# LockedFlysher/optimal_control_problem

Measured on AMD Instinct MI355X. Metric: QP solves/sec (batched OSQP-ADMM, N=20), higher is better.
Workload: dtype f64

## Files before the change

### __graft_entry__.py

```python
import os
import subprocess
import sys

ROOT = os.path.dirname(os.path.abspath(__file__))
if ROOT not in sys.path:
    sys.path.insert(0, ROOT)


def _run(cmd):
    subprocess.check_call(cmd, cwd=ROOT, stdout=subprocess.DEVNULL)


def _stale(target, deps):
    return (not os.path.exists(target)) or any(os.path.getmtime(d) > os.path.getmtime(target) for d in deps)


def build():
    pk = os.path.join(ROOT, "optimal_control_problem_amd")
    so = os.path.join(pk, "libmpcqp.so")
    cdir = os.path.join(pk, "csrc")
    csrc = [os.path.join(cdir, f) for f in sorted(os.listdir(cdir)) if f.endswith((".hip", ".hpp")) or f == "Makefile"]
    if _stale(so, csrc + [os.path.join(ROOT, "include", "mpcqp.h")]):
        _run(["make", "-C", cdir, "-j", str(min(8, os.cpu_count() or 1)), "../libmpcqp.so"])
    orc = os.path.join(ROOT, "oracle", "liborc.so")
    if _stale(orc, [os.path.join(ROOT, "oracle", "osqp_oracle.c"), os.path.join(ROOT, "oracle", "osqp_oracle.h")]):
        _run(["make", "-C", os.path.join(ROOT, "oracle"), "-B", "liborc.so"])
    pi = os.path.join(ROOT, "tests", "support", "libplan_interp.so")
    if _stale(pi, [os.path.join(ROOT, "tests", "support", "plan_interp.cpp"), os.path.join(pk, "csrc", "plan.hpp"), os.path.join(pk, "csrc", "select.hpp")]):
        _run(["g++", "-O2", "-std=c++17", "-fPIC", "-shared", "-o", pi, os.path.join(ROOT, "tests", "support", "plan_interp.cpp")])
    sm = os.path.join(ROOT, "tests", "support", "libstage_models_host.so")
    if _stale(sm, [os.path.join(ROOT, "tests", "support", "stage_models_host.cpp"), os.path.join(pk, "csrc", "stage_models.hpp")]):
        _run(["g++", "-O2", "-std=c++17", "-ffp-contract=off", "-fPIC", "-shared", "-o", sm, os.path.join(ROOT, "tests", "support", "stage_models_host.cpp")])
    st = os.path.join(ROOT, "tests", "support", "libstage_tracking_host.so")
    if _stale(st, [os.path.join(ROOT, "tests", "support", "stage_tracking_host.cpp"), os.path.join(pk, "csrc", "stage_models.hpp")]):
        _run(["g++", "-O2", "-std=c++17", "-ffp-contract=off", "-fPIC", "-shared", "-o", st, os.path.join(ROOT, "tests", "support", "stage_tracking_host.cpp")])
    sl_ = os.path.join(ROOT, "tests", "support", "libstage_link_cost_host.so")
    if _stale(sl_, [os.path.join(ROOT, "tests", "support", "stage_link_cost_host.cpp"), os.path.join(pk, "csrc", "stage_models.hpp")]):
        _run(["g++", "-O2", "-std=c++17", "-ffp-contract=off", "-fPIC", "-shared", "-o", sl_, os.path.join(ROOT, "tests", "support", "stage_link_cost_host.cpp")])
    cv = os.path.join(ROOT, "tests", "support", "libconvexify_host.so")
    if _stale(cv, [os.path.join(ROOT, "tests", "support", "convexify_host.cpp"), os.path.join(pk, "csrc", "stage_convexify.hpp"),
                   os.path.join(pk, "csrc", "stage_models.hpp"), os.path.join(ROOT, "include", "mpcqp.h")]):
        _run(["g++", "-O2", "-std=c++17", "-ffp-contract=off", "-fPIC", "-shared", "-o", cv, os.path.join(ROOT, "tests", "support", "convexify_host.cpp")])
    cpp = os.path.join(ROOT, "tests", "support", "cucaqp_cpp_test")
    src = os.path.join(ROOT, "tests", "support", "cucaqp_cpp_test.cpp")
# ... 84 lines not shown
```

### optimal_control_problem_amd/csrc/kernel_oc_rescale.hpp

```cpp
#pragma once

template <int NW, bool HUB>
__global__ void __launch_bounds__(NW * WAVE, 2) mpcqp_oc_rescale_kernel(const DevPlan pl, const DevRes rs, const mpcqp_settings st, const DevIO io, const DevOc oc) {
  extern __shared__ __attribute__((aligned(16))) double lds[];
  constexpr int NT = NW * WAVE;
  const int lane = threadIdx.x & 63;
  const int b = __builtin_amdgcn_readfirstlane(io.order ? io.order[blockIdx.x] : (int)blockIdx.x);
  int wid = __builtin_amdgcn_readfirstlane(threadIdx.x >> 6);
  if constexpr (NW == 4) wid = oc_wave_role4(lds, wid, lane, io.no_remap);
  const int tid = wid * WAVE + lane;
  const OcLds<NW> L = oc_lds<NW, true>(lds, pl, rs, oc);
  RCtx cx;
  cx.pl = &pl; cx.rs = &rs; cx.st = &st; cx.wid = wid; cx.lane = lane;
  cx.fts[0] = cx.fts[1] = cx.fts[2] = cx.fts[3] = 0;
  double *ws = io.ws + (long)b * pl.ws_stride; cx.ws = ws;
  cx.BL = ws + pl.o_Lf; cx.TMP = lds;
  cx.X = L.X; cx.Q = L.Q; cx.R = L.R; cx.Z = L.Z; cx.Y = L.Y; cx.W = L.W; cx.RB = L.RB; cx.RED = L.RED;
  double *valA = ws + pl.o_ellA, *valAt = ws + pl.o_ellAt, *valP = ws + pl.o_ellP;
  double *lb = ws + pl.o_l, *ub = ws + pl.o_u, *Qs = ws + pl.o_Lb;
  const double *Dg = ws + pl.o_D, *Eg = ws + pl.o_E;
  const double *inP = io.P + (long)b * io.sP, *inA = io.A + (long)b * io.sA, *inq = io.q + (long)b * io.sq;
  const double *inl = io.l + (long)b * io.sl, *inu = io.u + (long)b * io.su;
  const int n = pl.n, m = pl.m, npad = pl.npad, mpad = pl.mpad;
  cx.unscale = st.scaling && !st.scaled_termination;
// ... 12 lines not shown
    const int i = ch * WAVE + lane; const double ei = i < mpad ? cx.W[i] : 0.0;
    ell_map_chunk<true>(valA, pl.A.src, inA, pl.A.idx, valA, cx.coA[ch], cx.coA[ch + 1], lane, [&](double v, int j) { return v * (ei * cx.R[j]); });
  }
  for (int ch = wid; ch < pl.At.nchunks; ch += NW) {
    const int t = ch * WAVE + lane; const double dj = t < npad ? cx.R[t] : 0.0;
    ell_map_chunk<true>(valAt, pl.At.src, inA, pl.At.idx, valAt, cx.coAt[ch], cx.coAt[ch + 1], lane, [&](double v, int i) { return v * (dj * cx.W[i]); });
  }
  for (int ch = wid; ch < pl.P.nchunks; ch += NW) {
    const int t = ch * WAVE + lane; const double dj = t < npad ? cx.R[t] : 0.0;
    ell_map_chunk<true>(valP, pl.P.src, inP, pl.P.idx, valP, cx.coP[ch], cx.coP[ch + 1], lane, [&](double v, int k) { return v * (c * dj * cx.R[k]); });
  }
  bsync<NW>();
  double rho = io.info[4L * b + 3];
  if (!(rho >= Q_RHO_MIN && rho <= Q_RHO_MAX)) rho = fmin(fmax(st.rho, Q_RHO_MIN), Q_RHO_MAX);
  cx.rho = uni(rho);
  const bool ok = factorize_res<NW, (HUB ? 2 : 1), false>(cx, &oc, L.octab, lds);
  if (tid == 0) {
    io.status[b] = ok ? MPCQP_UNSOLVED : MPCQP_NON_CVX; io.iters[b] = 0;
    io.info[4L * b + 3] = cx.rho;
  }
}
```

### optimal_control_problem_amd/csrc/kernel_oc_split.hpp

```cpp
#pragma once

constexpr int OC_PENDING = 100, OC_PENDING_NONCVX = 101;
template <int NW>
struct OcLds {
  double *X, *Q, *R, *Z, *Y, *W, *RB, *RED;
  int *octab, *co;
};
template <int NW, bool SETUP = false>
__device__ __forceinline__ OcLds<NW> oc_lds(double *lds, const DevPlan &pl, const DevRes &rs, const DevOc &oc) {
  OcLds<NW> L;
  L.X = lds + rs.stage; L.Q = L.X + pl.npad; L.R = SETUP ? L.Q : L.Q + pl.npad;
  double *rend = L.R + pl.npad + rs.rext;
  L.Z = rend; L.Y = L.Z + (SETUP ? oc.zpad : pl.mpad); L.W = L.Y + (SETUP ? pl.npad : pl.mpad);
  L.RB = L.W + pl.mpad; L.RED = L.RB + 16 * NW + 16;
  L.octab = reinterpret_cast<int *>(L.RED + 16 * NW) + 8;
  L.co = L.octab + ((oc.o_pos + 1) & ~1);
  return L;
}
__device__ __forceinline__ int oc_wave_role4(double *lds, int wid, const int lane, const int no_remap) {
  const unsigned hw = __builtin_amdgcn_s_getreg((31 << 11) | 4), la = __builtin_amdgcn_s_getreg((31 << 11) | 6);
  const int simd = (hw >> 4) & 3, slot = (la & 0xff) != 0;
  int *xs = reinterpret_cast<int *>(lds);
  if (lane == 0) xs[wid] = simd;
  bsync<4>();
// ... 52 lines not shown
  double *lb = ws + pl.o_l, *ub = ws + pl.o_u, *Dg = ws + pl.o_D, *Eg = ws + pl.o_E, *Qs = ws + pl.o_Lb;
  const double *inP = io.P + (long)b * io.sP, *inA = io.A + (long)b * io.sA, *inq = io.q + (long)b * io.sq;
  const double *inl = io.l + (long)b * io.sl, *inu = io.u + (long)b * io.su;
  const int n = pl.n, m = pl.m, npad = pl.npad, mpad = pl.mpad;
  cx.unscale = st.scaling && !st.scaled_termination;
  TS_DECL;
#ifdef MPCQP_TIMING_RUIZ
  unsigned long long rzacc[5] = {0, 0, 0, 0, 0};
#endif
  if (oc.resume && io.status[b] != OC_PENDING) return;
  oc_tables_to_lds<NW>(pl, oc, cx, L, tid);
  if (oc.resume) {
    bsync<NW>();
    cx.rho = uni(io.info[4L * b + 3]);
    cx.c = 1.0; cx.cinv = 1.0;
    const bool okr = factorize_res<NW, (HUB ? 2 : 1), false>(cx, &oc, L.octab, lds);
    if (tid == 0) io.status[b] = okr ? OC_PENDING : OC_PENDING_NONCVX;
    return;
  }
  double c = 1.0;
  int refactor = 1, prev_status = MPCQP_UNSOLVED;
  const bool reuse = REUSE && io.reuse;
  if (reuse) {
    prev_status = io.status[b];
    c = io.cscale[b];
    for (int t = tid; t < npad; t += NT) { if (pl.perm[t] < 0) Qs[t] = 0.0; cx.R[t] = Dg[t]; }
    bsync<NW>();
    for (int j = tid; j < n; j += NT) { const int t = pl.pos[j]; Qs[t] = inq[j] * (c * cx.R[t]); }
    double chg[1] = {0.0};
    for (int i = tid; i < mpad; i += NT) {
      const double ei = Eg[i];
// ... 163 lines not shown
    };
    unsigned short *iA16 = reinterpret_cast<unsigned short *>(lds) + oc.ixo_a, *iP16 = reinterpret_cast<unsigned short *>(lds) + oc.ixo_p;
    constexpr std::false_type plain{}; constexpr std::true_type regs{};
    if (a_lds && p_lds && oc.ix16 == 3) scale_phase(lds, lds + pl.A.entries, iA16, iP16, plain);
    else if (a_lds && p_lds && oc.ix16 == 1) scale_phase(lds, lds + pl.A.entries, iA16, pl.P.idx, plain);
    else if (a_lds && p_lds) scale_phase(lds, lds + pl.A.entries, pl.A.idx, pl.P.idx, plain);
    else if (a_lds) scale_phase(lds, valP, pl.A.idx, pl.P.idx, regs);
    else if (oc.ix16 == 3) scale_phase(valA, valP, iA16, iP16, regs);
    else if (oc.ix16 == 1) scale_phase(valA, valP, iA16, pl.P.idx, regs);
    else scale_phase(valA, valP, pl.A.idx, pl.P.idx, regs);
  }
  bsync<NW>();
  cx.rho = uni(reuse ? io.info[4L * b + 3] : fmin(fmax(io.rho0 && io.rho0[b] > 0.0 ? io.rho0[b] : st.rho, Q_RHO_MIN), Q_RHO_MAX));
  TS(2);
  bool ok = !(reuse && prev_status == MPCQP_NON_CVX);
  if (ok && refactor) ok = factorize_res<NW, (HUB ? 2 : 1), false>(cx, &oc, L.octab, lds);
  if (tid == 0) {
    io.status[b] = ok ? MPCQP_UNSOLVED : MPCQP_NON_CVX; io.iters[b] = 0;
    io.info[4L * b + 3] = cx.rho;
    io.cscale[b] = c;
  }
  TS(3);
#ifdef MPCQP_TIMING
  ts_acc[12] = cx.fts[0]; ts_acc[13] = cx.fts[1]; ts_acc[14] = cx.fts[2]; ts_acc[15] = cx.fts[3];
#ifdef MPCQP_TIMING_RUIZ
  ts_acc[9] = rzacc[0]; ts_acc[10] = rzacc[1]; ts_acc[11] = rzacc[2]; ts_acc[12] = rzacc[3]; ts_acc[13] = rzacc[4];
#endif
#endif
  TS_STORE(io.dbg);
}

// ... 329 lines not shown
```

### optimal_control_problem_amd/csrc/kernel_onchip.hpp

```cpp
#pragma once

struct DevTile {
  int on, ntile;
  int nAr, nAtr;
  const int *Ar_off, *Ar_idx, *Ar_src, *Atr_off, *Atr_idx, *Atr_src;
  long Ar_entries, Atr_entries;
  const int *tJ, *rowid, *tsrc;
  const int *ta_info, *ta_cnt;
  const unsigned long long *ta_mask;
  const int *tt_info;
  long o_tile, o_ellAr, o_ellAtr;
};
struct DevOc {
  int nbc, has_hub, junc, npw, nhr, nlds, ntab;
  int o_chainE, o_chainF, o_pos, o_fill, ghub_slot, ghub_src;
  const int *a_assign;
  int npair, o_pair;
  int nfill, o_s, o_dbl, ndbl, o_pp;
  int at_poll, at_free;
  int a_lds, p_lds;
  const int *tab;
  const int *asm_rec;
  DevTile tl;
  int resume;
  int ixo_a, ixo_p;
  int ix16, zpad;
  int no_ruiz_regs = 0;
};

__host__ __device__ __forceinline__ int oc_swz(int r, int c) {
  return ((r ^ ((r >> 2) & 1)) << 4) | (c ^ (((r >> 1) & 3) << 2) ^ (((r >> 3) & 1) << 1));
}

typedef double d2 __attribute__((ext_vector_type(2)));

struct OcLane {
  unsigned f4;
  unsigned t4;
  int k4;
  int o4;
};
__device__ __forceinline__ OcLane oc_lane(int lane) {
  OcLane ln;
// ... 811 lines not shown
```

### optimal_control_problem_amd/csrc/kernel_resident.hpp

```cpp
#pragma once

#ifdef MPCQP_TIMING
#define TS_DECL unsigned long long ts_last = __builtin_amdgcn_s_memtime(), ts_acc[16] = {0}; const unsigned long long ts_first = ts_last, ts_rt0 = __builtin_amdgcn_s_memrealtime()
#define TS(k) do { unsigned long long t_ = __builtin_amdgcn_s_memtime(); ts_acc[k] += t_ - ts_last; ts_last = t_; } while (0)
#define TS_STORE(ptr) do { if (tid == 0 && (ptr)) { for (int k_ = 0; k_ < 16; k_++) (ptr)[16L * b + k_] = (long long)ts_acc[k_]; \
    if (b == 0) { (ptr)[16L * gridDim.x + 126] = (long long)(__builtin_amdgcn_s_memtime() - ts_first); (ptr)[16L * gridDim.x + 127] = (long long)(__builtin_amdgcn_s_memrealtime() - ts_rt0); } } } while (0)
#else
#define TS_DECL
#ifdef MPCQP_ASM_MARKS
#define TS(k) do { __builtin_amdgcn_sched_barrier(0); asm volatile("; TS " #k ::: "memory"); } while (0)
#else
#define TS(k) __builtin_amdgcn_sched_barrier(0)
#endif
#define TS_STORE(ptr)
#endif
struct DevRes {
  int nphase, ntemp, nconst, rext;
  const int *lv_ptr, *lv_diag, *lw_ptr, *lw_slot, *lw_g, *lu_ptr, *lu_dst, *lu_tmp, *lu_b, *g_ptr, *g_seg;
  int n_seg, nlev; long stage;
  int tmp_alias;
};


struct RCtx {
// ... 347 lines not shown
  t.i[0] = __builtin_amdgcn_mov_dpp(a.i[0], 0xB1, 0xF, 0xF, true);
  t.i[1] = __builtin_amdgcn_mov_dpp(a.i[1], 0xB1, 0xF, 0xF, true);
  a.d += t.d;
  t.i[0] = __builtin_amdgcn_mov_dpp(a.i[0], 0x4E, 0xF, 0xF, true);
  t.i[1] = __builtin_amdgcn_mov_dpp(a.i[1], 0x4E, 0xF, 0xF, true);
  return a.d + t.d;
}

__device__ __forceinline__ d4 mfma_abt_l(const double *A, const double *B, d4 acc, int lane) {
  const int rr = lane & 15, kk = lane >> 4;
#pragma unroll
  for (int k0 = 0; k0 < BS; k0 += 4) {
    const double a = A[rr * BS + k0 + kk];
    const double b = B[rr * BS + k0 + kk];
    acc = __builtin_amdgcn_mfma_f64_16x16x4f64(a, b, acc, 0, 0, 0);
  }
  return acc;
}

template <bool T>
__device__ __forceinline__ d4 load_blk(const char *BLb, const int off, const int offN, const int offT) {
  if (T) {
    const char *B = BLb + off + offT;
    d4 r;
    r[0] = *reinterpret_cast<const double *>(B); r[1] = *reinterpret_cast<const double *>(B + BS * 8);
    r[2] = *reinterpret_cast<const double *>(B + 2 * BS * 8); r[3] = *reinterpret_cast<const double *>(B + 3 * BS * 8);
    return r;
  }
  return *reinterpret_cast<const d4 *>(BLb + off + offN);
}
// ... 130 lines not shown
#pragma unroll
  for (int u = 0; u < U; u++) { v[u] = vp[u * WAVE]; fl[u] = fp[u * WAVE]; ix[u] = ip[u * WAVE]; }
#pragma unroll
  for (int u = 0; u < U; u++) if (fl[u]) acc += w[ix[u]] * v[u] * v[u];
  vp += U * WAVE; fp += U * WAVE; ip += U * WAVE;
}
template <int U>
__device__ __forceinline__ void tscatter_batch(const double *&vp, const int *&tp, double *T, const double sr) {
  double v[U]; int t[U];
#pragma unroll
  for (int u = 0; u < U; u++) { v[u] = vp[u * WAVE]; t[u] = tp[u * WAVE]; }
#pragma unroll
  for (int u = 0; u < U; u++) if (t[u] >= 0) T[t[u]] = v[u] * sr;
  vp += U * WAVE; tp += U * WAVE;
}
template <int NW, int OCM = 0, bool TAIL = true>
__device__ __forceinline__ bool factorize_res(RCtx &cx, const DevOc *oc = nullptr, const int *octab = nullptr, double *scr = nullptr) {
  const DevPlan &pl = *cx.pl; const DevRes &rs = *cx.rs; double *ws = cx.ws;
  const int wid = cx.wid, lane = cx.lane, tid = wid * WAVE + lane; constexpr int NT = NW * WAVE;
  const double *lb = ws + pl.o_l, *ub = ws + pl.o_u;
  const double *valA = ws + pl.o_ellA, *valAt = ws + pl.o_ellAt, *valP = ws + pl.o_ellP;
  double *T = ws + pl.o_T;
#ifdef MPCQP_TIMING
  unsigned long long f0 = __builtin_amdgcn_s_memtime();
#endif
  for (int i = tid; i < pl.mpad; i += NT) cx.W[i] = i < pl.m ? rho_of(lb[i], ub[i], cx.rho) : 0.0;
  bsync<NW>();
  {
    const double sigma = cx.st->sigma;
    const DevEll &E = pl.At;
    for (int c = wid; c < E.nchunks; c += NW) {
      double acc = 0.0;
      const int s0 = cx.coAt[c], s1 = cx.coAt[c + 1];
      const long o = (long)s0 * WAVE + lane;
      const double *vp = valAt + o; const int *fp = E.flag + o, *ip = E.idx + o;
      int rem = s1 - s0;
      for (; rem >= 8; rem -= 8) dvec_batch<8>(vp, fp, ip, cx.W, acc);
      if (rem & 4) dvec_batch<4>(vp, fp, ip, cx.W, acc);
      if (rem & 2) dvec_batch<2>(vp, fp, ip, cx.W, acc);
      if (rem & 1) dvec_batch<1>(vp, fp, ip, cx.W, acc);
      const int t = c * WAVE + lane;
      if (t < pl.npad) cx.R[t] = pl.perm[t] >= 0 ? sigma + acc : 1.0;
    }
  }
  {
    const DevEll &E = pl.A;
    for (int c = wid; c < E.nchunks; c += NW) {
      const int i = c * WAVE + lane;
      const double sr = sqrt(cx.W[i]);
      const int s0 = cx.coA[c], s1 = cx.coA[c + 1];
      const long o = (long)s0 * WAVE + lane;
      const double *vp = valA + o; const int *tp = pl.tpos + o;
      int rem = s1 - s0;
      for (; rem >= 8; rem -= 8) tscatter_batch<8>(vp, tp, T, sr);
      if (rem & 4) tscatter_batch<4>(vp, tp, T, sr);
      if (rem & 2) tscatter_batch<2>(vp, tp, T, sr);
      if (rem & 1) tscatter_batch<1>(vp, tp, T, sr);
    }
  }
  int *rec = nullptr;
  if constexpr (OCM > 0) {
    rec = reinterpret_cast<int *>(scr + OC_LDL_SCR * BLK);
    for (int k = tid; k < 8 * pl.nblk; k += NT) rec[k] = oc->asm_rec[k];
  }
  bsync<NW>();
#ifdef MPCQP_TIMING
  unsigned long long f1 = __builtin_amdgcn_s_memtime(); cx.fts[0] += f1 - f0;
#endif
  const int row0 = lane >> 4, col = lane & 15;
  if constexpr (OCM > 0) {
    const int nblk = pl.nblk;
    auto rfl = [](int v) { return __builtin_amdgcn_readfirstlane(v); };
    auto fetch_ops = [&](const int bb, d4 (&A)[3], d4 (&B)[3], int &n, int &J) {
      const int4 r0 = *reinterpret_cast<const int4 *>(rec + 8 * bb), r1 = *reinterpret_cast<const int4 *>(rec + 8 * bb + 4);
      n = rfl(r0.x); J = rfl(r0.y);
      const int o = (lane & 15) * BS + 4 * (lane >> 4);
      A[0] = *reinterpret_cast<const d4 *>(T + (long)rfl(r0.z) * BLK + o); B[0] = *reinterpret_cast<const d4 *>(T + (long)rfl(r0.w) * BLK + o);
      if (n > 1) { A[1] = *reinterpret_cast<const d4 *>(T + (long)rfl(r1.x) * BLK + o); B[1] = *reinterpret_cast<const d4 *>(T + (long)rfl(r1.y) * BLK + o); }
      if (n > 2) { A[2] = *reinterpret_cast<const d4 *>(T + (long)rfl(r1.z) * BLK + o); B[2] = *reinterpret_cast<const d4 *>(T + (long)rfl(r1.w) * BLK + o); }
    };
    auto fetch_pidx = [&](const int bb, int (&pi)[4]) {
#pragma unroll
      for (int g = 0; g < 4; g++) pi[g] = pl.asm_pidx[(long)bb * BLK + g * WAVE + lane];
    };
    if (wid < nblk) {
// ... 16 lines not shown
          if (mk[g]) acc[g] += pv[g];
          const int row = row0 + 4 * g;
          if (J >= 0 && row == col) acc[g] += cx.R[J * BS + row];
          cx.BL[(long)bb * BLK + row * BS + col] = acc[g];
        }
      };
      fetch_ops(wid, A0, B0, n0, J0); fetch_pidx(wid, pin);
      gather(pv0, m0); fetch_pidx(min(wid + NW, bl), pin);
      for (int b = wid; b < nblk; b += 2 * NW) {
        const int b1 = min(b + NW, bl), b2 = min(b + 2 * NW, bl), b3 = min(b + 3 * NW, bl);
        fetch_ops(b1, A1, B1, n1, J1); gather(pv1, m1); fetch_pidx(b2, pin);
        finish(b, A0, B0, n0, J0, pv0, m0);
        fetch_ops(b2, A0, B0, n0, J0); gather(pv0, m0); fetch_pidx(b3, pin);
        finish(b1, A1, B1, n1, J1, pv1, m1);
      }
    }
  } else {
  for (int b = wid; b < pl.nblk; b += NW) {
    d4 acc = {0, 0, 0, 0};
    for (int g = pl.asm_ptr[b]; g < pl.asm_ptr[b + 1]; g++) acc = mfma_abt_l(T + (long)pl.asm_a[g] * BLK, T + (long)pl.asm_b[g] * BLK, acc, lane);
    const int J = pl.blk_diag[b];
#pragma unroll
    for (int g = 0; g < 4; g++) {
      const int pi = pl.asm_pidx[(long)b * BLK + g * WAVE + lane];
      if (pi >= 0) acc[g] += valP[pi];
      const int row = row0 + 4 * g;
      if (J >= 0 && row == col) acc[g] += cx.R[J * BS + row];
      cx.BL[(long)b * BLK + row * BS + col] = acc[g];
    }
  }
// ... 609 lines not shown
```

### optimal_control_problem_amd/csrc/mpcqp.hip

```cpp
#include <map>
#include <mutex>
#include "kernels_all.hpp"
#include "kernels_util.hpp"
#include "reduced.hpp"

static_assert(SEL_ERR_ARG == MPCQP_ERR_ARG && SEL_ERR_LIMIT == MPCQP_ERR_LIMIT, "select.hpp reports its refusals in the codes of include/mpcqp.h");

static thread_local std::string g_last_error;
static int fail(int code, const std::string &msg) { g_last_error = msg; return code; }
int mpcqp_set_error(int code, const std::string &msg) { return fail(code, msg); }
int mpcqp_pick_device(int requested, int *device) {
  int ndev = 0;
  if (hipGetDeviceCount(&ndev) != hipSuccess || ndev <= 0) return fail(MPCQP_ERR_NO_GPU, "hipGetDeviceCount found no device");
  int dev = requested;
  if (dev < 0) { if (hipGetDevice(&dev) != hipSuccess) dev = 0; }
  if (dev >= ndev) return fail(MPCQP_ERR_ARG, "device ordinal out of range");
  hipDeviceProp_t prop;
  if (hipGetDeviceProperties(&prop, dev) != hipSuccess) return fail(MPCQP_ERR_HIP, "hipGetDeviceProperties failed");
  if (std::string(prop.gcnArchName).find("gfx950") == std::string::npos)
    return fail(MPCQP_ERR_NO_GPU, std::string("device is ") + prop.gcnArchName + ", kernels are built for gfx950 only");
  *device = dev;
  return MPCQP_OK;
}
#define HIPCHK(expr)                                                                              \
// ... 245 lines not shown
  for (size_t k = 0; k < (size_t)tp.ntile * BS; k++) if (tp.rowid[k] >= 0) mask[tp.rowid[k] / WAVE] |= 1ull << (tp.rowid[k] % WAVE);
  UP(upload(h, mask, &t.ta_mask));
  t.o_tile = s.wl.tile; t.o_ellAr = s.wl.ellAr; t.o_ellAtr = s.wl.ellAtr;
  return MPCQP_OK;
}
static int upload_onchip(mpcqp_handle *h, int cus) {
  Selection &s = h->sel; const Plan &pl = s.plan; const OcPlan &o = s.ocplan; const ResPlan &rp = s.rplan; DevRes &dr = h->dres; DevOc &d = h->doc;
  dr.stage = s.stage; dr.rext = oc_rext(rp.nw, std::max<int>(1, (int)o.pairs.size())); dr.nconst = 0; dr.n_seg = 0;
  d.nbc = o.nbc; d.has_hub = o.has_hub; d.junc = o.junc; d.npw = o.npw; d.nhr = o.nhr; d.nlds = o.nlds; d.ntab = (int)o.tab.size();
  d.o_chainE = o.o_chainE; d.o_chainF = o.o_chainF; d.o_pos = o.o_pos; d.o_fill = o.o_fill; d.ghub_slot = o.ghub_slot; d.ghub_src = o.ghub_src;
  d.npair = (int)o.pairs.size(); d.o_pair = o.o_pair; d.nfill = o.nfill; d.o_s = o.o_s; d.o_dbl = o.o_dbl; d.ndbl = (int)o.dbl.size(); d.o_pp = o.o_pp;
  d.at_poll = s.at_poll; d.at_free = s.at_free;
  d.a_lds = s.a_lds; d.p_lds = s.p_lds;
  if (s.vtiles && !mpcqp_kernel_oc_admm_tl(s.waves, s.oc_ng(), s.oc_nh())) s.vtiles = false;
  UP(upload(h, o.tab, &d.tab));
  UP(upload(h, oc_asm_records(pl), &d.asm_rec));
  if (s.tiles || s.vtiles) UP(upload_tiles(h));
  const SetupShape &su = s.setup; DevRes &ds = h->dres_setup; DevOc &dd = h->doc_setup;
  ds = dr; dd = d;
  dd.a_lds = su.a_lds; dd.p_lds = su.p_lds; dd.ix16 = su.ix16; dd.zpad = su.zpad; dd.ixo_a = su.ixo_a; dd.ixo_p = su.ixo_p;
  dd.no_ruiz_regs = h->knobs.no_ruiz_regs ? 1 : 0;
  ds.stage = su.stage;
  if (!s.split) return MPCQP_OK;
  if (s.oc8 && !s.vtiles && !s.a_assign.empty()) UP(upload(h, s.a_assign, &d.a_assign));
  if (s.oc8) {
    int nb = 0; h->qslots = 256;
    if (hipOccupancyMaxActiveBlocksPerMultiprocessor(&nb, oc_admm_of(h, false), s.waves * WAVE, (size_t)s.lds) == hipSuccess && nb > 0) {
      h->qslots = nb * (cus > 0 ? cus : 256);
    } else (void)hipGetLastError();
    UP(dalloc(h, &h->qctr, 16 * 16));
  }
  if (h->knobs.verbose) fprintf(stderr, "%s, %d resident workgroups\n", setup_shape_text(s).c_str(), h->qslots);
  return MPCQP_OK;
}
static int alloc_workspace(mpcqp_handle *h) {
  const size_t stride = (size_t)h->sel.wl.stride, batch = (size_t)h->batch; const int n = h->n, m = h->m;
// ... 679 lines not shown
```

### optimal_control_problem_amd/csrc/plan.hpp

```cpp
#pragma once
#include <algorithm>
#include <cstdint>
#include <map>
#include <set>
#include <string>
#include <utility>
#include <vector>

namespace mpcqp {

constexpr int BS = 16;
constexpr int BLK = BS * BS;
constexpr int WAVE = 64;

struct Ell {
  int nrows = 0, nchunks = 0;
  std::vector<int> chunk_off;
  std::vector<int> idx;
  std::vector<int> src;
  std::vector<int> flag;
  int slots() const { return chunk_off.empty() ? 0 : chunk_off.back(); }
  long entries() const { return (long)slots() * WAVE; }
};

// ... 890 lines not shown
    if (p0 >= oc.nbc) { if (fre >= 0) return; fre = c; }
    else if (p1 < oc.nbc && p0 > early) { if (poll >= 0) return; poll = c; }
    else return;
  }
  *at_poll = poll; *at_free = fre;
}
inline std::vector<int> oc_asm_records(const Plan &pl) {
  std::vector<int> r((size_t)8 * pl.nblk, std::max(pl.nT, 1));
  for (int b = 0; b < pl.nblk; b++) {
    const int p0 = pl.asm_ptr[b], n = pl.asm_ptr[b + 1] - p0;
    r[8 * b] = n; r[8 * b + 1] = pl.blk_diag[b];
    for (int t = 0; t < std::min(n, 3); t++) { r[8 * b + 2 + 2 * t] = pl.asm_a[p0 + t]; r[8 * b + 3 + 2 * t] = pl.asm_b[p0 + t]; }
  }
  return r;
}
inline long oc_stage_doubles(const OcPlan &oc, const ResPlan &rp, const Plan &pl) {
  return std::max((long)std::max(oc.nlds, rp.ntemp) * BLK, 8L * BLK + ((4L * pl.nblk + 15) / 16) * 16);
}
inline long lds_bytes_oc(const Plan &pl, const ResPlan &rp, const OcPlan &oc, bool zy_global = false, const TilePlan *tp = nullptr) {
  long tab_words = ((long)oc.o_pos + 1) / 2 + 4 + ((long)pl.A.nchunks + pl.At.nchunks + pl.P.nchunks + 3 + 1 + 1) / 2;
  if (tp && tp->on) tab_words += ((long)tp->Ar.nchunks + tp->Atr.nchunks + 2 + 1) / 2;
  return (oc_stage_doubles(oc, rp, pl) + 3L * pl.npad + oc_rext(rp.nw, std::max<int>(1, (int)oc.pairs.size())) + (zy_global ? 1L : 3L) * pl.mpad + 16L * rp.nw + 16 + 16L * rp.nw + tab_words) * 8L;
}

inline long lds_bytes(const Plan &pl) {
  const long tiles = pl.npad >= 2 * BS * (BS + 1) ? 0 : 2L * BS * (BS + 1);
  return (3L * pl.npad + 3L * pl.mpad + tiles + 64) * 8L;
}

}
// ... 1 lines not shown
```

### optimal_control_problem_amd/csrc/select.hpp

```cpp
#pragma once
#include <climits>
#include <cstdio>
#include <cstdlib>
#include <string>
#include <vector>

#include "plan.hpp"

namespace mpcqp {

constexpr int OC_NG = 5, OC_NH = 3;
struct Oc8Inst { int ng, nh; bool zyg; };
constexpr Oc8Inst OC8_INST[2] = {{4, 4, false}, {7, 7, false}};
constexpr long OC_LDS_MAX = 80 * 1024;
constexpr long OC8_LDS_MAX = 160 * 1024;
constexpr int OC8_MAX_CHAIN = 64;
constexpr long LDS_MAX = 160 * 1024;

constexpr int SEL_ERR_ARG = 1, SEL_ERR_LIMIT = 5;

struct Knobs {
  bool variant_named = false; std::string variant;
  bool autotune = false;
  bool verbose = false;
// ... 8 lines not shown
  bool oc_pad4 = false;
  bool no_zyg = false;
  bool gb_occ2 = false;
  bool gb_occ3 = false;
  bool no_res1x = false;
  bool no_res3 = false;
  bool pd4 = false;
  long lds_min = 0;
  int tiles = 0;
  int vtiles = 0;
  int doubles = -1;
  bool late = false;
  int resume_rounds = 1;
  bool no_ix16 = false;
  bool no_ruiz_regs = false;
  long setup_cap = LONG_MIN;
  bool no_abalance = false;
  bool no_touch = false;
  bool touch4 = false;
  bool touch8 = false;
  bool no_remap = false;
  int pipe_streams = 2;

  static Knobs from_env() {
    auto set = [](const char *name) { return getenv(name) != nullptr; };
    auto one = [](const char *name) { const char *e = getenv(name); return !e ? 0 : e[0] == '1' ? 2 : 1; };
    Knobs k;
    if (const char *e = getenv("MPCQP_VARIANT")) { k.variant_named = true; k.variant = e; }
    k.autotune = one("MPCQP_AUTOTUNE") == 2;
    k.verbose = set("MPCQP_VERBOSE");
// ... 8 lines not shown
    k.oc_pad4 = set("MPCQP_OC_PAD4");
    k.no_zyg = set("MPCQP_NO_ZYG");
    k.gb_occ2 = set("MPCQP_GB_OCC2");
    k.gb_occ3 = set("MPCQP_GB_OCC3");
    k.no_res1x = set("MPCQP_NO_RES1X");
    k.no_res3 = set("MPCQP_NO_RES3");
    k.pd4 = set("MPCQP_PD4");
    if (const char *e = getenv("MPCQP_LDS_MIN")) k.lds_min = atol(e);
    k.tiles = one("MPCQP_TILES");
    k.vtiles = one("MPCQP_VTILES");
    if (const char *e = getenv("MPCQP_DOUBLES")) k.doubles = std::max(0, atoi(e));
    k.late = set("MPCQP_LATE");
    if (const char *e = getenv("MPCQP_RESUME_ROUNDS")) k.resume_rounds = std::max(0, std::min(atoi(e), 8));
    k.no_ix16 = set("MPCQP_NO_IX16");
    k.no_ruiz_regs = one("MPCQP_NO_RUIZ_REGS") == 2;
    if (const char *e = getenv("MPCQP_SETUP_CAP")) k.setup_cap = atol(e);
    k.no_abalance = set("MPCQP_NO_ABALANCE");
    k.no_touch = set("MPCQP_NO_TOUCH");
    k.touch4 = set("MPCQP_TOUCH4");
    k.touch8 = set("MPCQP_TOUCH8");
    k.no_remap = set("MPCQP_NO_REMAP");
    if (const char *e = getenv("MPCQP_PIPE_STREAMS")) k.pipe_streams = std::max(1, std::min(atoi(e), 8));
    return k;
  }
};

struct SetupShape {
  int nw = 0; long lds = 0, stage = 0;
  int a_lds = 0, p_lds = 0, ix16 = 0, zpad = 0, ixo_a = 0, ixo_p = 0;
  long vecs = 0, tabw = 0;
};

struct Selection {
  int err = 0; std::string error;
  int waves = 0;
  bool wide = false;
  bool gblocks = false;
  bool zyg = false;
  bool occ3 = false;
  bool occ4 = false;
  bool res1x = false;
  int res3 = 0;
  bool stream_pd8 = false;
  bool oc = false;
  int oc8 = 0;
  bool split = false;
  bool tiles = false;
  bool vtiles = false;
  int resume_rounds = 1;
  Plan plan; ResPlan rplan; OcPlan ocplan; TilePlan tplan; WsLayout wl;
  long lds = 0;
  long stage = 0;
  int a_lds = 0, p_lds = 0;
  int at_poll = -1, at_free = -1;
  SetupShape setup;
  std::vector<int> a_assign;

  int family() const { return oc ? 200 + waves : gblocks ? 100 + waves : waves; }
  int oc_ng() const { return oc8 > 0 ? OC8_INST[oc8 - 1].ng : OC_NG; }
  int oc_nh() const { return !ocplan.has_hub ? 0 : oc8 > 0 ? OC8_INST[oc8 - 1].nh : OC_NH; }
};

namespace sel {

struct Ctx {
// ... 197 lines not shown
      auto z_fits = [&](long z) { return total + z <= cap && cu / ((total + z) * 8) == cu / (total * 8); };
      if (a_scr && z_fits(zP)) { r.ix16 = 3; r.ixo_a = 0; r.zpad = (int)zP; r.ixo_p = (int)(4 * (r.stage + zoff)); }
      else if (p_scr && z_fits(zA)) { r.ix16 = 3; r.ixo_p = 0; r.zpad = (int)zA; r.ixo_a = (int)(4 * (r.stage + zoff)); }
      else if (a_scr) { r.ix16 = 1; r.ixo_a = 0; }
      else if (z_fits(zA)) { r.ix16 = 1; r.zpad = (int)zA; r.ixo_a = (int)(4 * (r.stage + zoff)); }
      total += r.zpad;
    }
    r.bytes = total * 8; r.fits = total <= cap;
    return r;
  };
  Shape sh = shape(cu / 2);
  if (c.k.setup_cap != LONG_MIN) sh = shape(c.k.setup_cap);
  else { const Shape s3 = shape(cu / 3); if (s3.fits && (s3.a || !(sh.a && sh.p))) sh = s3; }
  su.a_lds = sh.a; su.p_lds = sh.p; su.ix16 = sh.ix16; su.zpad = sh.zpad; su.ixo_a = sh.ixo_a; su.ixo_p = sh.ixo_p;
  su.stage = sh.stage; su.nw = 4; su.lds = sh.bytes; su.vecs = vec + sh.zpad; su.tabw = tabw;
  if (s.oc8 && !c.k.no_abalance) {
    std::vector<int> assign(8 * 32, -1), load(8, 0), cnt(8, 0), order_(pq.A.nchunks);
    for (int ch = 0; ch < pq.A.nchunks; ch++) order_[ch] = ch;
    auto batches = [&](int ch) { return ell_batches8(pq.A.chunk_off[ch + 1] - pq.A.chunk_off[ch]); };
    std::stable_sort(order_.begin(), order_.end(), [&](int a, int b) { return batches(a) > batches(b); });
    bool okA = true;
    for (int ch : order_) {
      int w = 0;
      for (int v = 1; v < 8; v++) if (load[v] < load[w] || (load[v] == load[w] && cnt[v] < cnt[w])) w = v;
      if (cnt[w] >= 32) { okA = false; break; }
      assign[w * 32 + cnt[w]++] = ch; load[w] += std::max(1, batches(ch));
    }
    if (okA) s.a_assign = assign;
  }
}
// ... 108 lines not shown
```

Baseline: 1.087 million.

## Stage T tiles in swizzled LDS and use singleton lists in setup factorization

```diff
diff --git a/__graft_entry__.py b/__graft_entry__.py
--- a/__graft_entry__.py
+++ b/__graft_entry__.py
@@ -28,6 +28,9 @@
     pi = os.path.join(ROOT, "tests", "support", "libplan_interp.so")
     if _stale(pi, [os.path.join(ROOT, "tests", "support", "plan_interp.cpp"), os.path.join(pk, "csrc", "plan.hpp"), os.path.join(pk, "csrc", "select.hpp")]):
         _run(["g++", "-O2", "-std=c++17", "-fPIC", "-shared", "-o", pi, os.path.join(ROOT, "tests", "support", "plan_interp.cpp")])
+    tl = os.path.join(ROOT, "tests", "support", "libt_lds_interp.so")
+    if _stale(tl, [os.path.join(ROOT, "tests", "support", "t_lds_interp.cpp"), os.path.join(pk, "csrc", "plan.hpp"), os.path.join(pk, "csrc", "select.hpp")]):
+        _run(["g++", "-O2", "-std=c++17", "-fPIC", "-shared", "-o", tl, os.path.join(ROOT, "tests", "support", "t_lds_interp.cpp")])
     sm = os.path.join(ROOT, "tests", "support", "libstage_models_host.so")
     if _stale(sm, [os.path.join(ROOT, "tests", "support", "stage_models_host.cpp"), os.path.join(pk, "csrc", "stage_models.hpp")]):
         _run(["g++", "-O2", "-std=c++17", "-ffp-contract=off", "-fPIC", "-shared", "-o", sm, os.path.join(ROOT, "tests", "support", "stage_models_host.cpp")])
diff --git a/optimal_control_problem_amd/csrc/kernel_oc_rescale.hpp b/optimal_control_problem_amd/csrc/kernel_oc_rescale.hpp
--- a/optimal_control_problem_amd/csrc/kernel_oc_rescale.hpp
+++ b/optimal_control_problem_amd/csrc/kernel_oc_rescale.hpp
@@ -50,7 +50,7 @@
   double rho = io.info[4L * b + 3];
   if (!(rho >= Q_RHO_MIN && rho <= Q_RHO_MAX)) rho = fmin(fmax(st.rho, Q_RHO_MIN), Q_RHO_MAX);
   cx.rho = uni(rho);
-  const bool ok = factorize_res<NW, (HUB ? 2 : 1), false>(cx, &oc, L.octab, lds);
+  const bool ok = factorize_res<NW, (HUB ? 2 : 1), false, true>(cx, &oc, L.octab, lds);
   if (tid == 0) {
     io.status[b] = ok ? MPCQP_UNSOLVED : MPCQP_NON_CVX; io.iters[b] = 0;
     io.info[4L * b + 3] = cx.rho;
diff --git a/optimal_control_problem_amd/csrc/kernel_oc_split.hpp b/optimal_control_problem_amd/csrc/kernel_oc_split.hpp
--- a/optimal_control_problem_amd/csrc/kernel_oc_split.hpp
+++ b/optimal_control_problem_amd/csrc/kernel_oc_split.hpp
@@ -90,7 +90,7 @@
     bsync<NW>();
     cx.rho = uni(io.info[4L * b + 3]);
     cx.c = 1.0; cx.cinv = 1.0;
-    const bool okr = factorize_res<NW, (HUB ? 2 : 1), false>(cx, &oc, L.octab, lds);
+    const bool okr = factorize_res<NW, (HUB ? 2 : 1), false, true>(cx, &oc, L.octab, lds);
     if (tid == 0) io.status[b] = okr ? OC_PENDING : OC_PENDING_NONCVX;
     return;
   }
@@ -284,7 +284,7 @@
   cx.rho = uni(reuse ? io.info[4L * b + 3] : fmin(fmax(io.rho0 && io.rho0[b] > 0.0 ? io.rho0[b] : st.rho, Q_RHO_MIN), Q_RHO_MAX));
   TS(2);
   bool ok = !(reuse && prev_status == MPCQP_NON_CVX);
-  if (ok && refactor) ok = factorize_res<NW, (HUB ? 2 : 1), false>(cx, &oc, L.octab, lds);
+  if (ok && refactor) ok = factorize_res<NW, (HUB ? 2 : 1), false, true>(cx, &oc, L.octab, lds);
   if (tid == 0) {
     io.status[b] = ok ? MPCQP_UNSOLVED : MPCQP_NON_CVX; io.iters[b] = 0;
     io.info[4L * b + 3] = cx.rho;
diff --git a/optimal_control_problem_amd/csrc/kernel_onchip.hpp b/optimal_control_problem_amd/csrc/kernel_onchip.hpp
--- a/optimal_control_problem_amd/csrc/kernel_onchip.hpp
+++ b/optimal_control_problem_amd/csrc/kernel_onchip.hpp
@@ -14,6 +14,7 @@
 struct DevOc {
   int nbc, has_hub, junc, npw, nhr, nlds, ntab;
   int o_chainE, o_chainF, o_pos, o_fill, ghub_slot, ghub_src;
+  int su_path;
   const int *a_assign;
   int npair, o_pair;
   int nfill, o_s, o_dbl, ndbl, o_pp;
@@ -27,6 +28,7 @@
   int ix16, zpad;
   int no_ruiz_regs = 0;
 };
+static_assert(sizeof(DevOc) == 312 && offsetof(DevOc, a_assign) == 56, "DevOc is a kernel argument of every on-chip instance: its layout is part of their text");
 
 __host__ __device__ __forceinline__ int oc_swz(int r, int c) {
   return ((r ^ ((r >> 2) & 1)) << 4) | (c ^ (((r >> 1) & 3) << 2) ^ (((r >> 3) & 1) << 1));
diff --git a/optimal_control_problem_amd/csrc/kernel_resident.hpp b/optimal_control_problem_amd/csrc/kernel_resident.hpp
--- a/optimal_control_problem_amd/csrc/kernel_resident.hpp
+++ b/optimal_control_problem_amd/csrc/kernel_resident.hpp
@@ -385,6 +385,15 @@
     const double a = A[rr * BS + k0 + kk];
     const double b = B[rr * BS + k0 + kk];
     acc = __builtin_amdgcn_mfma_f64_16x16x4f64(a, b, acc, 0, 0, 0);
+  }
+  return acc;
+}
+__device__ __forceinline__ d4 mfma_abt_tl(const double *A, const double *B, d4 acc, int lane) {
+  const int rr = lane & 15, kk = lane >> 4;
+#pragma unroll
+  for (int k0 = 0; k0 < BS; k0 += 4) {
+    const int o = t_lds_off(rr, k0 + kk);
+    acc = __builtin_amdgcn_mfma_f64_16x16x4f64(A[o], B[o], acc, 0, 0, 0);
   }
   return acc;
 }
@@ -545,7 +554,7 @@
   for (int u = 0; u < U; u++) if (t[u] >= 0) T[t[u]] = v[u] * sr;
   vp += U * WAVE; tp += U * WAVE;
 }
-template <int NW, int OCM = 0, bool TAIL = true>
+template <int NW, int OCM = 0, bool TAIL = true, bool SU = false>
 __device__ __forceinline__ bool factorize_res(RCtx &cx, const DevOc *oc = nullptr, const int *octab = nullptr, double *scr = nullptr) {
   const DevPlan &pl = *cx.pl; const DevRes &rs = *cx.rs; double *ws = cx.ws;
   const int wid = cx.wid, lane = cx.lane, tid = wid * WAVE + lane; constexpr int NT = NW * WAVE;
@@ -556,8 +565,54 @@
   unsigned long long f0 = __builtin_amdgcn_s_memtime();
 #endif
   for (int i = tid; i < pl.mpad; i += NT) cx.W[i] = i < pl.m ? rho_of(lb[i], ub[i], cx.rho) : 0.0;
+  [[maybe_unused]] const int *sut = nullptr, *suh = nullptr;
+  [[maybe_unused]] bool t_lds = false, d_list = false;
+  [[maybe_unused]] auto t_zero = [&](const int p) {
+    const int nd = sut[suh[5] + 8 * p + 2];
+    int t0 = tid; asm volatile("" : "+v"(t0));
+    for (int k = t0; 2 * k < nd; k += NT) reinterpret_cast<d2 *>(scr)[k] = d2{0.0, 0.0};
+  };
+  [[maybe_unused]] auto t_scatter = [&](const int p) {
+    const int2 *sc = reinterpret_cast<const int2 *>(sut + sut[suh[5] + 8 * p + 3]);
+    const int cnt = sut[suh[5] + 8 * p + 4];
+    int k = tid; asm volatile("" : "+v"(k));
+    for (; k + 3 * NT < cnt; k += 4 * NT) {
+      int2 e[4]; double v[4];
+#pragma unroll
+      for (int u = 0; u < 4; u++) e[u] = sc[k + u * NT];
+#pragma unroll
+      for (int u = 0; u < 4; u++) v[u] = valA[e[u].x];
+#pragma unroll
+      for (int u = 0; u < 4; u++) scr[(unsigned)e[u].y & 0xffffu] = v[u] * sqrt(cx.W[(unsigned)e[u].y >> 16]);
+    }
+    for (; k < cnt; k += NT) { const int2 e = sc[k]; scr[(unsigned)e.y & 0xffffu] = valA[e.x] * sqrt(cx.W[(unsigned)e.y >> 16]); }
+  };
+  if constexpr (SU) {
+    sut = oc->asm_rec; suh = sut + 8 * pl.nblk;
+    t_lds = OCM > 0 && (oc->su_path & 1); d_list = (oc->su_path & 2) != 0;
+    if (t_lds) t_zero(0);
+  }
   bsync<NW>();
-  {
+  if (SU && d_list) {
+    if constexpr (SU) {
+      const double sigma = cx.st->sigma;
+      const int K = suh[6], np = pl.npad;
+      const int *se = sut + suh[7], *sr = se + K * np;
+      for (int c = wid; c < pl.At.nchunks; c += NW) {
+        const int t = c * WAVE + lane;
+        if (t < np) {
+          double acc = 0.0;
+          for (int k = 0; k < K; k += 2) {
+            const int e0 = se[k * np + t], e1 = se[(k + 1) * np + t], r0 = sr[k * np + t], r1 = sr[(k + 1) * np + t];
+            const double v0 = valAt[max(e0, 0)], v1 = valAt[max(e1, 0)], w0 = cx.W[max(r0, 0)], w1 = cx.W[max(r1, 0)];
+            if (e0 >= 0) acc = __builtin_fma(w0 * v0, v0, acc);
+            if (e1 >= 0) acc = __builtin_fma(w1 * v1, v1, acc);
+          }
+          cx.R[t] = pl.perm[t] >= 0 ? sigma + acc : 1.0;
+        }
+      }
+    }
+  } else {
     const double sigma = cx.st->sigma;
     const DevEll &E = pl.At;
     for (int c = wid; c < E.nchunks; c += NW) {
@@ -574,7 +629,9 @@
       if (t < pl.npad) cx.R[t] = pl.perm[t] >= 0 ? sigma + acc : 1.0;
     }
   }
-  {
+  if (SU && t_lds) {
+    if constexpr (SU) t_scatter(0);
+  } else {
     const DevEll &E = pl.A;
     for (int c = wid; c < E.nchunks; c += NW) {
       const int i = c * WAVE + lane;
@@ -592,6 +649,11 @@
   int *rec = nullptr;
   if constexpr (OCM > 0) {
     rec = reinterpret_cast<int *>(scr + OC_LDL_SCR * BLK);
+    if constexpr (SU) {
+      const int *src = oc->asm_rec;
+      if (t_lds) { rec = reinterpret_cast<int *>(scr + suh[1]); src = sut + suh[2]; }
+      for (int k = tid; k < 8 * pl.nblk; k += NT) rec[k] = src[k];
+    } else
     for (int k = tid; k < 8 * pl.nblk; k += NT) rec[k] = oc->asm_rec[k];
   }
   bsync<NW>();
@@ -600,6 +662,62 @@
 #endif
   const int row0 = lane >> 4, col = lane & 15;
   if constexpr (OCM > 0) {
+    if (SU && t_lds) {
+      if constexpr (SU) {
+        auto rfl = [](int v) { return __builtin_amdgcn_readfirstlane(v); };
+        const int ol = t_lds_off(lane & 15, 4 * (lane >> 4));
+        auto lds_tile = [&](const int slot) {
+          const double *q = scr + slot * BLK;
+          const d2 lo = *reinterpret_cast<const d2 *>(q + ol), hi = *reinterpret_cast<const d2 *>(q + (ol ^ 2));
+          return d4{lo[0], lo[1], hi[0], hi[1]};
+        };
+        int pin[4];
+        auto fetch_pidx = [&](const int bb) {
+#pragma unroll
+          for (int g = 0; g < 4; g++) pin[g] = pl.asm_pidx[(long)bb * BLK + g * WAVE + lane];
+        };
+        auto gather = [&](double (&pv)[4], bool (&mk)[4]) {
+#pragma unroll
+          for (int g = 0; g < 4; g++) { pv[g] = valP[max(pin[g], 0)]; mk[g] = pin[g] >= 0; }
+        };
+        auto finish = [&](const int bb, const double (&pv)[4], const bool (&mk)[4]) {
+          const int4 r0 = *reinterpret_cast<const int4 *>(rec + 8 * bb), r1 = *reinterpret_cast<const int4 *>(rec + 8 * bb + 4);
+          const int n = rfl(r0.x), J = rfl(r0.y);
+          d4 acc = {0, 0, 0, 0};
+          acc = oc_mm(lds_tile(rfl(r0.z)), lds_tile(rfl(r0.w)), acc);
+          if (n > 1) acc = oc_mm(lds_tile(rfl(r1.x)), lds_tile(rfl(r1.y)), acc);
+          if (n > 2) acc = oc_mm(lds_tile(rfl(r1.z)), lds_tile(rfl(r1.w)), acc);
+          if (n > 3) {
+            const int *ta = sut + suh[3], *tb = sut + suh[4];
+            for (int g = pl.asm_ptr[bb] + 3; g < pl.asm_ptr[bb + 1]; g++) acc = mfma_abt_tl(scr + ta[g] * BLK, scr + tb[g] * BLK, acc, lane);
+          }
+#pragma unroll
+          for (int g = 0; g < 4; g++) {
+            if (mk[g]) acc[g] += pv[g];
+            const int row = row0 + 4 * g;
+            if (J >= 0 && row == col) acc[g] += cx.R[J * BS + row];
+            cx.BL[(long)bb * BLK + row * BS + col] = acc[g];
+          }
+        };
+        const int parts = suh[0];
+        for (int p = 0; p < parts; p++) {
+          if (p > 0) { bsync<NW>(); t_zero(p); bsync<NW>(); t_scatter(p); bsync<NW>(); }
+          const int b1 = sut[suh[5] + 8 * p + 1], bw = sut[suh[5] + 8 * p] + wid;
+          if (bw < b1) {
+            const int bl = bw + (b1 - 1 - bw) / NW * NW;
+            double pv0[4], pv1[4]; bool m0[4], m1[4];
+            fetch_pidx(bw); gather(pv0, m0); fetch_pidx(min(bw + NW, bl));
+            for (int b = bw; b < b1; b += 2 * NW) {
+              const int c1 = min(b + NW, bl), c2 = min(b + 2 * NW, bl), c3 = min(b + 3 * NW, bl);
+              gather(pv1, m1); fetch_pidx(c2);
+              finish(b, pv0, m0);
+              gather(pv0, m0); fetch_pidx(c3);
+              finish(c1, pv1, m1);
+            }
+          }
+        }
+      }
+    } else {
     const int nblk = pl.nblk;
     auto rfl = [](int v) { return __builtin_amdgcn_readfirstlane(v); };
     auto fetch_ops = [&](const int bb, d4 (&A)[3], d4 (&B)[3], int &n, int &J) {
@@ -646,6 +764,7 @@
         fetch_ops(b2, A0, B0, n0, J0); gather(pv0, m0); fetch_pidx(b3, pin);
         finish(b1, A1, B1, n1, J1, pv1, m1);
       }
+    }
     }
   } else {
   for (int b = wid; b < pl.nblk; b += NW) {
diff --git a/optimal_control_problem_amd/csrc/mpcqp.hip b/optimal_control_problem_amd/csrc/mpcqp.hip
--- a/optimal_control_problem_amd/csrc/mpcqp.hip
+++ b/optimal_control_problem_amd/csrc/mpcqp.hip
@@ -283,12 +283,13 @@
   d.a_lds = s.a_lds; d.p_lds = s.p_lds;
   if (s.vtiles && !mpcqp_kernel_oc_admm_tl(s.waves, s.oc_ng(), s.oc_nh())) s.vtiles = false;
   UP(upload(h, o.tab, &d.tab));
-  UP(upload(h, oc_asm_records(pl), &d.asm_rec));
+  UP(upload(h, oc_setup_tables(pl, s.tlds, s.sing), &d.asm_rec));
   if (s.tiles || s.vtiles) UP(upload_tiles(h));
   const SetupShape &su = s.setup; DevRes &ds = h->dres_setup; DevOc &dd = h->doc_setup;
   ds = dr; dd = d;
   dd.a_lds = su.a_lds; dd.p_lds = su.p_lds; dd.ix16 = su.ix16; dd.zpad = su.zpad; dd.ixo_a = su.ixo_a; dd.ixo_p = su.ixo_p;
   dd.no_ruiz_regs = h->knobs.no_ruiz_regs ? 1 : 0;
+  dd.su_path = (s.split && su.t_parts > 0 ? 1 : 0) | (s.split && su.sing_k > 0 ? 2 : 0);
   ds.stage = su.stage;
   if (!s.split) return MPCQP_OK;
   if (s.oc8 && !s.vtiles && !s.a_assign.empty()) UP(upload(h, s.a_assign, &d.a_assign));
diff --git a/optimal_control_problem_amd/csrc/plan.hpp b/optimal_control_problem_amd/csrc/plan.hpp
--- a/optimal_control_problem_amd/csrc/plan.hpp
+++ b/optimal_control_problem_amd/csrc/plan.hpp
@@ -928,6 +928,93 @@
   }
   return r;
 }
+constexpr int t_lds_off(int r, int c) { return r * BS + ((((c >> 1) ^ (r >> 1) ^ ((((r >> 1) + 2) >> 1) & 2)) << 1) | (c & 1)); }
+constexpr int T_LDS_MAX_PARTS = 8;
+struct TLdsPlan {
+  int parts = 0;
+  long cap = 0;
+  int rec_off = 0;
+  std::vector<int> blk0;
+  std::vector<int> image;
+  std::vector<int> sc_ptr;
+  std::vector<int> sc;
+  std::vector<int> rec;
+  std::vector<int> ta, tb;
+  std::vector<std::vector<int>> tiles;
+};
+inline TLdsPlan build_t_lds_plan(const Plan &pl, long stage, int max_parts = T_LDS_MAX_PARTS) {
+  TLdsPlan tp;
+  const long rec_off = stage + pl.npad - 4L * pl.nblk;
+  if (pl.nT <= 0 || rec_off < 2L * BLK || (rec_off & 1) || pl.mpad > 65536 || rec_off > 65536) return tp;
+  const int cap_tiles = (int)(rec_off / BLK);
+  std::vector<int> blk0{0}, slot_of(pl.nT, -1);
+  std::vector<std::vector<int>> tiles(1);
+  std::vector<int> rec = oc_asm_records(pl), ta(pl.asm_a.size()), tb(pl.asm_b.size());
+  for (int b = 0; b < pl.nblk; b++) {
+    const int g0 = pl.asm_ptr[b], g1 = pl.asm_ptr[b + 1];
+    auto missing = [&]() { std::set<int> s; for (int g = g0; g < g1; g++) for (int t : {pl.asm_a[g], pl.asm_b[g]}) if (slot_of[t] < 0) s.insert(t); return s; };
+    std::set<int> add = missing();
+    if (1 + (int)tiles.back().size() + (int)add.size() > cap_tiles) {
+      if (blk0.back() == b) return tp;
+      for (int t : tiles.back()) slot_of[t] = -1;
+      blk0.push_back(b); tiles.emplace_back();
+      add = missing();
+      if (1 + (int)add.size() > cap_tiles) return tp;
+    }
+    for (int t : add) { tiles.back().push_back(t); slot_of[t] = (int)tiles.back().size(); }
+    for (int g = g0; g < g1; g++) { ta[g] = slot_of[pl.asm_a[g]]; tb[g] = slot_of[pl.asm_b[g]]; }
+    for (int k = 2; k < 8; k++) rec[8 * b + k] = 0;
+    for (int g = g0; g < std::min(g1, g0 + 3); g++) { rec[8 * b + 2 + 2 * (g - g0)] = ta[g]; rec[8 * b + 3 + 2 * (g - g0)] = tb[g]; }
+  }
+  blk0.push_back(pl.nblk);
+  const int parts = (int)tiles.size();
+  if (parts > max_parts) return tp;
+  tp.sc_ptr.assign(1, 0);
+  for (int p = 0; p < parts; p++) {
+    std::fill(slot_of.begin(), slot_of.end(), -1);
+    for (size_t k = 0; k < tiles[p].size(); k++) slot_of[tiles[p][k]] = (int)k + 1;
+    for (int c = 0; c < pl.A.nchunks; c++) for (int s = pl.A.chunk_off[c]; s < pl.A.chunk_off[c + 1]; s++) for (int lane = 0; lane < WAVE; lane++) {
+      const long e = (long)s * WAVE + lane;
+      const int tq = pl.tpos[e];
+      if (tq < 0 || slot_of[tq / BLK] < 0) continue;
+      const int off = slot_of[tq / BLK] * BLK + t_lds_off((tq % BLK) / BS, tq % BS);
+      tp.sc.push_back((int)e); tp.sc.push_back((int)(((unsigned)(c * WAVE + lane) << 16) | (unsigned)off));
+    }
+    tp.sc_ptr.push_back((int)tp.sc.size() / 2);
+    tp.image.push_back((1 + (int)tiles[p].size()) * BLK);
+  }
+  tp.parts = parts; tp.cap = (long)cap_tiles * BLK; tp.rec_off = (int)rec_off;
+  tp.blk0 = blk0; tp.rec = rec; tp.ta = ta; tp.tb = tb; tp.tiles = tiles;
+  return tp;
+}
+struct SingList { int K = 0; std::vector<int> ent, row; };
+inline SingList build_sing_list(const Plan &pl) {
+  SingList sl;
+  std::vector<std::vector<int>> of(pl.npad);
+  for (int t = 0; t < pl.npad && t < pl.At.nchunks * WAVE; t++)
+    for (int s = pl.At.chunk_off[t / WAVE]; s < pl.At.chunk_off[t / WAVE + 1]; s++) { const long e = (long)s * WAVE + t % WAVE; if (pl.At.flag[e]) of[t].push_back((int)e); }
+  for (const auto &v : of) sl.K = std::max(sl.K, (int)v.size());
+  sl.K = (sl.K + 1) / 2 * 2;
+  sl.ent.assign((size_t)sl.K * pl.npad, -1); sl.row.assign((size_t)sl.K * pl.npad, -1);
+  for (int t = 0; t < pl.npad; t++) for (size_t k = 0; k < of[t].size(); k++) { sl.ent[k * pl.npad + t] = of[t][k]; sl.row[k * pl.npad + t] = pl.At.idx[of[t][k]]; }
+  return sl;
+}
+inline std::vector<int> oc_setup_tables(const Plan &pl, const TLdsPlan &tp, const SingList &sl) {
+  std::vector<int> r = oc_asm_records(pl);
+  const size_t h = r.size();
+  r.resize(h + 16, 0);
+  auto put = [&](const std::vector<int> &v) { if (r.size() & 1) r.push_back(0); const int o = (int)r.size(); r.insert(r.end(), v.begin(), v.end()); return o; };
+  r[h] = tp.parts; r[h + 1] = tp.rec_off; r[h + 6] = sl.K;
+  if (sl.K > 0) { const int o = put(sl.ent); put(sl.row); r[h + 7] = o; }
+  if (tp.parts > 0) {
+    const int o_rec = put(tp.rec), o_ta = put(tp.ta), o_tb = put(tp.tb), o_sc = put(tp.sc);
+    std::vector<int> pr((size_t)8 * tp.parts, 0);
+    for (int p = 0; p < tp.parts; p++) { int *q = &pr[8 * p]; q[0] = tp.blk0[p]; q[1] = tp.blk0[p + 1]; q[2] = tp.image[p]; q[3] = o_sc + 2 * tp.sc_ptr[p]; q[4] = tp.sc_ptr[p + 1] - tp.sc_ptr[p]; }
+    const int o_part = put(pr);
+    r[h + 2] = o_rec; r[h + 3] = o_ta; r[h + 4] = o_tb; r[h + 5] = o_part;
+  }
+  return r;
+}
 inline long oc_stage_doubles(const OcPlan &oc, const ResPlan &rp, const Plan &pl) {
   return std::max((long)std::max(oc.nlds, rp.ntemp) * BLK, 8L * BLK + ((4L * pl.nblk + 15) / 16) * 16);
 }
diff --git a/optimal_control_problem_amd/csrc/select.hpp b/optimal_control_problem_amd/csrc/select.hpp
--- a/optimal_control_problem_amd/csrc/select.hpp
+++ b/optimal_control_problem_amd/csrc/select.hpp
@@ -46,6 +46,8 @@
   int resume_rounds = 1;
   bool no_ix16 = false;
   bool no_ruiz_regs = false;
+  bool no_t_lds = false;
+  bool no_sing_list = false;
   long setup_cap = LONG_MIN;
   bool no_abalance = false;
   bool no_touch = false;
@@ -84,6 +86,8 @@
     if (const char *e = getenv("MPCQP_RESUME_ROUNDS")) k.resume_rounds = std::max(0, std::min(atoi(e), 8));
     k.no_ix16 = set("MPCQP_NO_IX16");
     k.no_ruiz_regs = one("MPCQP_NO_RUIZ_REGS") == 2;
+    k.no_t_lds = one("MPCQP_NO_T_LDS") == 2;
+    k.no_sing_list = one("MPCQP_NO_SING_LIST") == 2;
     if (const char *e = getenv("MPCQP_SETUP_CAP")) k.setup_cap = atol(e);
     k.no_abalance = set("MPCQP_NO_ABALANCE");
     k.no_touch = set("MPCQP_NO_TOUCH");
@@ -99,6 +103,7 @@
   int nw = 0; long lds = 0, stage = 0;
   int a_lds = 0, p_lds = 0, ix16 = 0, zpad = 0, ixo_a = 0, ixo_p = 0;
   long vecs = 0, tabw = 0;
+  int t_parts = 0, sing_k = 0;
 };
 
 struct Selection {
@@ -119,6 +124,7 @@
   bool vtiles = false;
   int resume_rounds = 1;
   Plan plan; ResPlan rplan; OcPlan ocplan; TilePlan tplan; WsLayout wl;
+  TLdsPlan tlds; SingList sing;
   long lds = 0;
   long stage = 0;
   int a_lds = 0, p_lds = 0;
@@ -346,6 +352,9 @@
   else { const Shape s3 = shape(cu / 3); if (s3.fits && (s3.a || !(sh.a && sh.p))) sh = s3; }
   su.a_lds = sh.a; su.p_lds = sh.p; su.ix16 = sh.ix16; su.zpad = sh.zpad; su.ixo_a = sh.ixo_a; su.ixo_p = sh.ixo_p;
   su.stage = sh.stage; su.nw = 4; su.lds = sh.bytes; su.vecs = vec + sh.zpad; su.tabw = tabw;
+  if (!c.k.no_t_lds) s.tlds = build_t_lds_plan(pq, su.stage);
+  if (!c.k.no_sing_list) s.sing = build_sing_list(pq);
+  su.t_parts = s.tlds.parts; su.sing_k = s.sing.K;
   if (s.oc8 && !c.k.no_abalance) {
     std::vector<int> assign(8 * 32, -1), load(8, 0), cnt(8, 0), order_(pq.A.nchunks);
     for (int ch = 0; ch < pq.A.nchunks; ch++) order_[ch] = ch;
```

Result: faster. 1.127 million (median of 6 runs) (+3.7%).
